# ntnu-arl/aerial_gym_simulator

Measured on AMD Instinct MI355X. Metric: env-steps/sec at N_envs=8192 per GPU (dynamics-only), higher is better.
Workload: dtype f32; 1 GPU; base_quadrotor position_setpoint_task, lee_position_control, empty_env, 1 sub-step/step (BASELINE configs[1]); num_envs_per_gpu=8192, num_envs_total=8192, rng=sync-free (device Philox4x32-10)

## Files before the change

aerial_gym_simulator_amd/csrc/agx_dynamics.hip:

```cpp
#include "agx_common.h"
#ifndef AGX_DYN_CONTRACT
#define AGX_DYN_CONTRACT 0
#endif
#ifndef AGX_DYN_WAVES
#define AGX_DYN_WAVES 3
#endif
#ifndef AGX_DYN_WAVES_LEAN_LAWS
#define AGX_DYN_WAVES_LEAN_LAWS 4
#endif
#ifndef AGX_DYN_WAVES_LOOP
#define AGX_DYN_WAVES_LOOP 2
#endif
#if AGX_DYN_CONTRACT
#pragma clang fp contract(fast)
#else
#pragma clang fp contract(off)
#endif
#include "agx_device_math.h"
#include "agx_nav_parts.h"
#include "agx_quad_math.h"
#include "agx_rng.h"
#include "agx_step_signal.h"

#include <chrono>
// ... 561 lines not shown
      }
      const bool any_dist = !body_wrench && (B.disturb != nullptr || B.disturb_prob > 0.0f);
      const bool split_root = !root_link && has_drag && any_dist;
      float dr[6] = {0.0f, 0.0f, 0.0f, 0.0f, 0.0f, 0.0f}, di[6] = {0.0f, 0.0f, 0.0f, 0.0f, 0.0f, 0.0f};
      if (has_drag) {
        float vbn = norm(d.vbody);
        dr[0] = (-P.lin_drag_linear[0] * d.vbody.x) + (-P.lin_drag_quadratic[0] * vbn * d.vbody.x);
        dr[1] = (-P.lin_drag_linear[1] * d.vbody.y) + (-P.lin_drag_quadratic[1] * vbn * d.vbody.y);
        dr[2] = (-P.lin_drag_linear[2] * d.vbody.z) + (-P.lin_drag_quadratic[2] * vbn * d.vbody.z);
        dr[3] = (-P.ang_drag_linear[0] * d.wbody.x) + (-P.ang_drag_quadratic[0] * fabsf(d.wbody.x) * d.wbody.x);
        dr[4] = (-P.ang_drag_linear[1] * d.wbody.y) + (-P.ang_drag_quadratic[1] * fabsf(d.wbody.y) * d.wbody.y);
        dr[5] = (-P.ang_drag_linear[2] * d.wbody.z) + (-P.ang_drag_quadratic[2] * fabsf(d.wbody.z) * d.wbody.z);
      }
      if (B.disturb) {
        const float *dd = B.disturb + (size_t)(sub_base + sub) * 7 * n + i;
        float occ = dd[0];
#pragma unroll
        for (int c = 0; c < 6; ++c) {
          float lo = -B.disturb_max[c], hi = B.disturb_max[c];
          di[c] = ((hi - lo) * dd[(size_t)(1 + c) * n] + lo) * occ;
        }
      } else if (B.disturb_prob > 0.0f) {
        float ud[7];
        rng_fill<7>(B.rng_seed, B.env_index_base + i, agx::step_index(B), RNG_DISTURB + sub_base + sub, ud);
        float occ = ud[0] < B.disturb_prob ? 1.0f : 0.0f;
#pragma unroll
        for (int c = 0; c < 6; ++c) {
          float lo = -B.disturb_max[c], hi = B.disturb_max[c];
          di[c] = ((hi - lo) * ud[1 + c] + lo) * occ;
        }
      }
      if (!body_wrench && (has_drag || any_dist)) {
#pragma unroll
        for (int c = 0; c < 6; ++c) bw[c] = split_root ? bw[c] + (dr[c] + di[c]) : (bw[c] + dr[c]) + di[c];
      }
      if (B.body_force && sub == k - 1) {
        AGX_AT(B.body_force, 0) = bw[0]; AGX_AT(B.body_force, 1) = bw[1]; AGX_AT(B.body_force, 2) = bw[2];
      }
      integrate(P, s, V3{bw[0], bw[1], bw[2]}, V3{bw[3], bw[4], bw[5]});
      if (B.boxes) {
        traj[(sub * 3 + 0) * bd + tid] = s.p.x;
        traj[(sub * 3 + 1) * bd + tid] = s.p.y;
        traj[(sub * 3 + 2) * bd + tid] = s.p.z;
        if (sub == 0) { tlo = s.p; thi = s.p; }
        tlo = V3{fminf(tlo.x, s.p.x), fminf(tlo.y, s.p.y), fminf(tlo.z, s.p.z)};
        thi = V3{fmaxf(thi.x, s.p.x), fmaxf(thi.y, s.p.y), fmaxf(thi.z, s.p.z)};
      }
    }
    bool crashed = crashed_in != 0;
    if (B.boxes && k > 0) crashed = collide_trajectory(B.boxes, B.num_boxes, n, i, traj, k, bd, tid, tlo, thi, P.collision_radius) || crashed;
    store_state(B.state, n, i, s);
    if (k > 0) {
      if (lean) store_body_velocities(B.derived, n, i, d);
      else store_derived(B.derived, n, i, d);
#pragma unroll
      for (int j = 0; j < M; ++j) AGX_AT(B.motor_thrust, j) = u[j];
      if (B.wrench_cmd) {
        AGX_AT(B.wrench_cmd, 0) = wc.f.x; AGX_AT(B.wrench_cmd, 1) = wc.f.y; AGX_AT(B.wrench_cmd, 2) = wc.f.z;
        AGX_AT(B.wrench_cmd, 3) = wc.t.x; AGX_AT(B.wrench_cmd, 4) = wc.t.y; AGX_AT(B.wrench_cmd, 5) = wc.t.z;
      }
    }
    float a_cur[AGX_MAX_ACTIONS], a_prev[AGX_MAX_ACTIONS];
#pragma unroll
    for (int c = 0; c < AGX_MAX_ACTIONS; ++c) {
      a_cur[c] = (k > 0 && !EXT) ? a_in[c] : a_old[c];
      a_prev[c] = (k >= 2 && !EXT) ? a_in[c] : ((k == 1 && !EXT) ? a_old[c] : a_prev_in[c]);
      if (c < A && k > 0 && !EXT && !lean) {
        AGX_AT(B.prev_actions, c) = a_prev[c];
        AGX_AT(B.actions, c) = a_cur[c];
      }
    }
    const int steps = steps_in + (more_launches ? 0 : 1);
    if (!more_launches) B.sim_steps[i] = steps;
    bool trunc = false;
    if (task_epilogue) {
      float rew;
      if (T.kind == AGX_TASK_POSITION) {
        rew = reward_position(s, d.qveh, d.wbody, tgt, crashed);
      } else {
        AGX_AT(T.prev_pos_err, 0) = ppe.x; AGX_AT(T.prev_pos_err, 1) = ppe.y; AGX_AT(T.prev_pos_err, 2) = ppe.z;
        V3 pe = quat_rotate_inverse(d.qveh, tgt - s.p);
        AGX_AT(T.pos_err, 0) = pe.x; AGX_AT(T.pos_err, 1) = pe.y; AGX_AT(T.pos_err, 2) = pe.z;
        rew = reward_navigation(T.rp, T.curriculum_progress, pe, ppe, a_cur[0], a_cur[2], a_cur[3], a_prev[0], a_prev[2],
                                a_prev[3], crashed);
      }
      T.reward[i] = rew;
      trunc = steps > T.episode_len;
      reset = (crashed && T.reset_on_collision) || trunc;
      B.reset_mask[i] = reset ? 1 : 0;
      if (T.successes) nav_bookkeeping_epilogue(T, i, true, tgt, s.p, crashed, trunc);
    }
    B.crashes[i] = crashed ? 1 : 0;
    if (!more_launches) B.truncations[i] = trunc ? 1 : 0;
  }
  if (T.kind != AGX_TASK_NONE && __ballot(reset) != 0ull && (tid & 63) == 0) atomicOr(B.reset_flag + B.flag_parity, 1);
  if (blockIdx.x == 0 && tid < 64) push_wait_finish(B, push_peek);
}

namespace q4 = quad;
AGX_DEV unsigned long long vote(bool p) { return __builtin_amdgcn_ballot_w64(p); }

struct QuadDerived {
  float euler, qveh, vveh, vbody, wbody;
};
AGX_DEV QuadDerived update_states_quad(float q, float v, float w, float extra, float &esn, float &ecs) {
  const int l = q4::lane_in_quad();
  QuadDerived d;
  const float e = q4::euler_xyz_0_2pi(q);
  d.euler = ssa(e);
  float sy, cy;
  const float half_yaw = (q4::bc<2>(e) * 1.0f) * 0.5f;
  sincos_bounded(l < 2 ? extra : half_yaw, sy, cy);
  esn = sy;
  ecs = cy;
  d.qveh = l == 2 ? sy : (l == 3 ? cy : 0.0f);
  d.vveh = q4::quat_rotate_inverse(d.qveh, v);
  d.vbody = q4::quat_rotate_inverse(q, v);
  d.wbody = q4::quat_rotate_inverse(q, w);
  return d;
}
AGX_DEV QuadDerived update_states_quad(float q, float v, float w) {
  float sn, cs;
  return update_states_quad(q, v, w, 0.0f, sn, cs);
}

template <int M>
struct QuadConsts {
  float grav, in0, in1, in2, ii0, ii1, ii2, pinv[M / 4][6], mapf[M], mapt[M], mass, dt;
};
template <int M>
AGX_DEV QuadConsts<M> load_quad_consts(const AgxRobotParams &P, const AgxRobotParams &S, int l, int l3) {
  QuadConsts<M> C;
  C.grav = P.gravity[l3];
  C.in0 = P.inertia[3 * l3 + 0]; C.in1 = P.inertia[3 * l3 + 1]; C.in2 = P.inertia[3 * l3 + 2];
  C.ii0 = P.inertia_inv[3 * l3 + 0]; C.ii1 = P.inertia_inv[3 * l3 + 1]; C.ii2 = P.inertia_inv[3 * l3 + 2];
#pragma unroll
  for (int h = 0; h < M / 4; ++h)
#pragma unroll
    for (int c = 0; c < 6; ++c) C.pinv[h][c] = P.alloc_pinv[6 * (l + 4 * h) + c];
  const float *wmap = S.root_link_mode != 0 ? P.alloc : P.wrench_map;
#pragma unroll
  for (int j = 0; j < M; ++j) {
    C.mapf[j] = wmap[M * l3 + j];
    C.mapt[j] = wmap[M * (3 + l3) + j];
  }
  C.mass = S.mass;
  C.dt = S.dt;
  return C;
}
template <int M>
AGX_DEV QuadConsts<M> load_quad_consts(const AgxRobotParams &P, int l, int l3) {
  return load_quad_consts<M>(P, P, l, l3);
}
AGX_DEV float quad_thrust_along_body_z(float q, float f, int l) {
  const float t1 = q * q4::bc<2>(q), t2 = q4::perm<1, 0, 2, 3>(q) * q4::bc<3>(q);
  const float c2a = 2.0f * (l == 1 ? t1 - t2 : t1 + t2);
  const float sqq = q * q;
  const float m22 = 1.0f - 2.0f * (q4::bc<0>(sqq) + q4::bc<1>(sqq));
  return q4::dot3(f, l == 2 ? m22 : c2a);
}
AGX_DEV float quad_desired_orientation_pos_vel_sc(float f, float sy, float cy, int l) {
  const float b3 = fdiv(f, q4::norm3(f));
  const float tmp = l == 0 ? cy : (l == 1 ? sy : 0.0f);
  const float cb = q4::cross3(b3, tmp);
  const float b2 = fdiv(cb, q4::norm3(cb));
  const float b1 = q4::cross3(b2, b3);
  return q4::rotmat_cols_to_quat(b1, b2, b3);
}
AGX_DEV float quad_desired_orientation_pos_vel(float f, float yaw, int l) {
  float sy, cy;
  sincos_bounded(yaw, sy, cy);
  return quad_desired_orientation_pos_vel_sc(f, sy, cy, l);
}
template <bool ZERO_RATE, int M>
AGX_DEV float quad_body_torque(const QuadConsts<M> &C, float q, float qd, float wb, float wsp, float kr, float kw, int l) {
  const float qe = q4::quat_mul(q4::conj(q), qd);
  const float pp = q4::rot1(qe) * q4::rot2(qe);
  const float pw = qe * q4::bc<3>(qe);
  const float mp = 2.0f * (pp + pw);
  const float mm = 2.0f * (pp - pw);
  const float rot_err = 0.5f * (l == 1 ? mm - mp : -(mp - mm));
  const float jw = (C.in0 * q4::bc<0>(wb) + C.in1 * q4::bc<1>(wb)) + C.in2 * q4::bc<2>(wb);
  const float ff = q4::cross3(wb, jw);
  const float we = ZERO_RATE ? wb : wb - q4::quat_rotate(qe, wsp);
  return ((-kr) * rot_err - kw * we) + ff;
}
template <int M>
AGX_DEV void quad_allocate(const AgxRobotParams &P, const QuadConsts<M> &C, float force, float torque, float (&u)[M / 4],
                           const float (&kT)[M / 4], const float (&tinc)[M / 4], const float (&tdec)[M / 4], float &fb, float &tb) {
  const float w0 = q4::bc<0>(force), w1 = q4::bc<1>(force), w2 = q4::bc<2>(force);
  const float w3 = q4::bc<0>(torque), w4 = q4::bc<1>(torque), w5 = q4::bc<2>(torque);
#pragma unroll
  for (int h = 0; h < M / 4; ++h) {
    float r = 0.0f;
    r += C.pinv[h][0] * w0;
    r += C.pinv[h][1] * w1;
    r += C.pinv[h][2] * w2;
    r += C.pinv[h][3] * w3;
    r += C.pinv[h][4] * w4;
    r += C.pinv[h][5] * w5;
    u[h] = motor_update(P, r, u[h], kT[h], tinc[h], tdec[h]);
  }
  fb = 0.0f;
  tb = 0.0f;
#pragma unroll
  for (int h = 0; h < M / 4; ++h) {
    const float u0 = q4::bc<0>(u[h]), u1 = q4::bc<1>(u[h]), u2 = q4::bc<2>(u[h]), u3 = q4::bc<3>(u[h]);
    fb += C.mapf[4 * h + 0] * u0; fb += C.mapf[4 * h + 1] * u1; fb += C.mapf[4 * h + 2] * u2; fb += C.mapf[4 * h + 3] * u3;
    tb += C.mapt[4 * h + 0] * u0; tb += C.mapt[4 * h + 1] * u1; tb += C.mapt[4 * h + 2] * u2; tb += C.mapt[4 * h + 3] * u3;
  }
}
template <int M>
AGX_DEV void quad_integrate(const AgxRobotParams &P, const QuadConsts<M> &C, float &p, float &q, float &v, float &w, float fb, float tb,
                            int l) {
  const float dt = C.dt;
  const float fw = q4::quat_rotate(q, fb);
  const float wbi = q4::quat_rotate_inverse(q, w);
  const float jwi = (C.in0 * q4::bc<0>(wbi) + C.in1 * q4::bc<1>(wbi)) + C.in2 * q4::bc<2>(wbi);
  const float rhs = tb - q4::cross3(wbi, jwi);
  const float dwb = (C.ii0 * q4::bc<0>(rhs) + C.ii1 * q4::bc<1>(rhs)) + C.ii2 * q4::bc<2>(rhs);
  const float wb_new = wbi + dt * dwb;
  float w_new = q4::quat_rotate(q, wb_new);
  float v_new = v + dt * fdiv(fw, C.mass);
  v_new = v_new + C.grav * dt;
  const float ml = fmaxf(1.0f - P.linear_damping * dt, 0.0f);
  const float ma = fmaxf(1.0f - P.angular_damping * dt, 0.0f);
  v_new = v_new * ml;
  w_new = w_new * ma;
  const float v2 = q4::dot3(v_new, v_new), w2 = q4::dot3(w_new, w_new);
  if (v2 > P.max_linear_velocity * P.max_linear_velocity) v_new = v_new * fdiv(P.max_linear_velocity, fsqrt(v2));
  if (w2 > P.max_angular_velocity * P.max_angular_velocity) w_new = w_new * fdiv(P.max_angular_velocity, fsqrt(w2));
  p = p + v_new * dt;
  const float wm2 = q4::dot3(w_new, w_new);
  if (wm2 != 0.0f) {
    const float wm = fsqrt(wm2);
    const float half = dt * wm * 0.5f;
    float sn, cs;
    sincos_bounded(half, sn, cs);
    const float sc = fdiv(sn, wm);
    const float x1 = w_new * sc;
    const float r3 = (x1 * q4::bc<3>(q) + q4::rot1(x1) * q4::rot2(q)) - q4::rot2(x1) * q4::rot1(q);
    const float xq = x1 * q;
    const float rw = (-q4::bc<0>(xq) - q4::bc<1>(xq)) - q4::bc<2>(xq);
    float rq = l == 3 ? rw : r3;
    rq += q * cs;
    const float nn = fsqrt(q4::dot4(rq, rq));
    q = fdiv(rq, nn);
  }
  v = v_new;
  w = w_new;
}

AGX_DEV float euler_rates_to_body_rates_quad(float euler, float rz) {
  const int l = q4::lane_in_quad();
  float sn, cs;
  sincos_bounded(euler, sn, cs);
  const float sr = q4::bc<0>(sn), cr = q4::bc<0>(cs), sp = q4::bc<1>(sn), cp = q4::bc<1>(cs);
  const float m0 = q4::by_lane(l, 1.0f, 0.0f, 0.0f);
  const float m1 = q4::by_lane(l, 0.0f, cr, -sr);
  const float m2 = q4::by_lane(l, -sp, sr * cp, cr * cp);
  return (m0 * 0.0f + m1 * 0.0f) + m2 * rz;
}
AGX_DEV float quat_from_euler_quad(float ang) {
  const int l = q4::lane_in_quad();
  float sn, cs;
  sincos_bounded(ang * 0.5f, sn, cs);
  const float sr = q4::bc<0>(sn), cr = q4::bc<0>(cs), sp = q4::bc<1>(sn), cp = q4::bc<1>(cs), sy = q4::bc<2>(sn), cy = q4::bc<2>(cs);
  const float a1 = l == 2 ? sy : cy, b1 = l == 0 ? sr : cr, c1 = l == 1 ? sp : cp;
  const float a2 = l == 2 ? cy : sy, b2 = l == 0 ? cr : sr, c2 = l == 1 ? cp : sp;
  const float t1 = a1 * b1 * c1, t2 = a2 * b2 * c2;
  return (l == 0 || l == 2) ? t1 - t2 : t1 + t2;
}

template <int CTRL, int M>
AGX_DEV void quad_controller(const AgxRobotParams &P, const QuadConsts<M> &C, float p, float q, float v, const QuadDerived &d, float a,
                             float a2, float kp, float kv, float kr, float kw, int l, float &force, float &torque) {
  const float yaw = q4::bc<2>(d.euler);
  float fz = 0.0f;
  if (CTRL == AGX_CTRL_FULLY_ACTUATED) {
    float nq = sqrtf(q4::dot4(a2, a2));
    nq = nq < 1e-9f ? 1e-9f : nq;
    const float qd = a2 / nq;
    const float acc = kp * (a - p) + kv * (0.0f - v);
    const float f = (acc - C.grav) * C.mass;
    force = q4::quat_rotate_inverse(q, f);
    torque = quad_body_torque<true>(C, q, qd, d.wbody, 0.0f, kr, kw, l);
    return;
  }
  if (CTRL == AGX_CTRL_POSITION || CTRL == AGX_CTRL_VELOCITY || CTRL == AGX_CTRL_VEL_STEERING) {
    float acc;
    if (CTRL == AGX_CTRL_POSITION) {
      acc = kp * (a - p) + kv * (0.0f - v);
    } else {
      const float sp_vel_w = q4::quat_rotate(d.qveh, a);
      acc = kp * (p - p) + kv * (sp_vel_w - v);
    }
    const float f = (acc - C.grav) * C.mass;
    fz = quad_thrust_along_body_z(q, f, l);
    const float qd = quad_desired_orientation_pos_vel(f, CTRL == AGX_CTRL_VELOCITY ? yaw : q4::bc<3>(a), l);
    if (CTRL == AGX_CTRL_POSITION) {
      torque = quad_body_torque<true>(C, q, qd, d.wbody, 0.0f, kr, kw, l);
    } else {
      float wsp = euler_rates_to_body_rates_quad(d.euler, CTRL == AGX_CTRL_VELOCITY ? q4::bc<3>(a) : 0.0f);
      if (l == 2) wsp = fminf(fmaxf(wsp, -P.max_yaw_rate), P.max_yaw_rate);
      torque = quad_body_torque<false>(C, q, qd, d.wbody, wsp, kr, kw, l);
    }
// ... 891 lines not shown
      if (l < 3) {
        AGX_QAT(B.derived, 0, ol) = d.euler;
        AGX_QAT(B.derived, 7, ol) = d.vveh;
        AGX_QAT(B.derived, 10, ol) = d.vbody;
        AGX_QAT(B.derived, 13, ol) = d.wbody;
      }
      AGX_QAT(B.derived, 3, ol) = d.qveh;
    }
    vbody = d.vbody;
    wbody = d.wbody;
  }
  if (valid) {
    float *o = obs + (size_t)i * 13;
    const float e = tgt - p;
    if (l < 3) { o[l] = e; o[7 + l] = vbody; o[10 + l] = wbody; }
    o[3 + l] = q;
    if (rows) {
      float *r = rows + (size_t)i * 16;
      if (B.push_world > 0) {
        const float e1 = q4::bc<1>(e), e2 = q4::bc<2>(e), q2 = q4::perm<0, 2, 2, 3>(q), q3 = q4::bc<3>(q);
        const float vb0 = q4::bc<0>(vbody), vb1 = q4::bc<1>(vbody), wb0 = q4::bc<0>(wbody), wb1 = q4::bc<1>(wbody), wb2 = q4::bc<2>(wbody);
        float t1 = 0.0f, t2 = 0.0f, t3 = 0.0f;
        if (l == 3) {
          t1 = tail_reward;
          t2 = tail_crashed ? 1.0f : 0.0f;
          t3 = tail_truncated ? 1.0f : 0.0f;
        }
        const float x0 = q4::by_lane(l, e, q, vb1, wb2);
        const float x1 = q4::by_lane(l, e1, q2, vbody, t1);
        const float x2 = q4::by_lane(l, e2, q3, wb0, t2);
        const float x3 = q4::by_lane(l, q, vb0, wb1, t3);
        row_store4_push(B, r + 4 * l, x0, x1, x2, x3);
      } else {
        if (l < 3) { row_store(B, r + l, e); row_store(B, r + 7 + l, vbody); row_store(B, r + 10 + l, wbody); }
        row_store(B, r + 3 + l, q);
        if (l == 0) {
          row_store(B, r + 13, tail_reward);
          row_store(B, r + 14, tail_crashed ? 1.0f : 0.0f);
          row_store(B, r + 15, tail_truncated ? 1.0f : 0.0f);
        }
      }
    }
  }
  step_rows_signal(B);
}
__global__ void __launch_bounds__(64, 1) k_reset_masked_quad_obs(AgxRobotParams P, AgxEnvBuffers B, int n, AgxResetArgs R,
                                                                 const float *__restrict__ target, float *__restrict__ obs) {
  reset_masked_quad_obs_body<false>(P, B, n, R, target, obs);
}
__global__ void __launch_bounds__(64, 1) k_reset_masked_quad_obs_host_draws(AgxRobotParams P, AgxEnvBuffers B, int n, AgxResetArgs R,
                                                                            const float *__restrict__ target,
                                                                            float *__restrict__ obs) {
  reset_masked_quad_obs_body<true>(P, B, n, R, target, obs);
}

#ifdef AGX_STEP_STAMPS
constexpr int kStampBlocks = 1024, kStampWords = 8;
__device__ unsigned long long g_step_stamps[kStampBlocks * 2 * kStampWords];
AGX_DEV void step_stamp(int k) {
  const unsigned long long t = k < 6 ? (unsigned long long)clock64() : (unsigned long long)wall_clock64();
  if ((threadIdx.x & 63u) == 0u && blockIdx.x < (unsigned)kStampBlocks)
    g_step_stamps[((size_t)blockIdx.x * 2 + (threadIdx.x >> 6)) * kStampWords + k] = t;
}
#define AGX_STAMP(k) step_stamp(k)
#define AGX_STAMP_ARRIVED(k) do { __builtin_amdgcn_s_waitcnt(0); step_stamp(k); } while (0)
#else
#define AGX_STAMP(k) do { } while (0)
#define AGX_STAMP_ARRIVED(k) do { } while (0)
#endif

AGX_DEV unsigned proof_key(float x) { return x >= 0.0f ? __float_as_uint(x) : 0x7FC00000u; }

__host__ __device__ inline unsigned proof_witness_bit(int episode_len, int reset_on_collision, int steps, float dist, float speed, float dt,
                                                      float vmax, float dv) {
  const int k = episode_len - steps + 1;
  if (k < 1 || k > AGX_PROOF_HORIZON || !(dist == dist) || !(speed == speed)) return 0u;
  bool w = k == 1 || !reset_on_collision;
  if (!w) {
    const float m = (float)(k - 1);
    const float travel = m * dt * fminf(vmax, speed + m * dv);
    w = dist + (travel * 1.01f + 1.0e-3f) < 8.0f;
  }
  return w ? (1u << k) : 0u;
}

template <bool MAX>
AGX_DEV unsigned wave_reduce_dpp(unsigned x) {
#define AGX_RED(ctrl)                                                                        \
  {                                                                                           \
    const unsigned y_ = (unsigned)__builtin_amdgcn_mov_dpp((int)x, (ctrl), 0xF, 0xF, true);   \
    x = MAX ? max(x, y_) : (x | y_);                                                          \
  }
  AGX_RED(0xB1)
  AGX_RED(0x4E)
  AGX_RED(0x124)
  AGX_RED(0x128)
#undef AGX_RED
  const unsigned r0 = (unsigned)__builtin_amdgcn_readlane((int)x, 0), r1 = (unsigned)__builtin_amdgcn_readlane((int)x, 16);
  const unsigned r2 = (unsigned)__builtin_amdgcn_readlane((int)x, 32), r3 = (unsigned)__builtin_amdgcn_readlane((int)x, 48);
  return MAX ? max(max(r0, r1), max(r2, r3)) : ((r0 | r1) | (r2 | r3));
}

AGX_DEV void proof_store_slot(const AgxTaskArgs &T, const AgxEnvBuffers &B, int wb, int nb, bool reset, unsigned horizon, int steps,
                              float dist, float speed) {
  const unsigned ar = wave_reduce_dpp<false>(reset ? 1u : 0u), hz = wave_reduce_dpp<false>(horizon);
  const unsigned ms = wave_reduce_dpp<true>((unsigned)max(steps, 0)), db = wave_reduce_dpp<true>(proof_key(dist));
  const unsigned vb = wave_reduce_dpp<true>(proof_key(speed));
  if ((threadIdx.x & 63u) == 0u) {
    uint4 *slot = reinterpret_cast<uint4 *>(T.proof_slots + ((size_t)(B.step_counter & 1) * nb + wb) * AGX_PROOF_SLOT_WORDS);
    slot[0] = make_uint4(((unsigned)B.step_counter + 1u) & 0x7FFFFFFFu, ar | (T.proof_mode == AGX_STEP_ANY ? 2u : 0u), hz, ms);
    slot[1] = make_uint4(db, vb, 0u, 0u);
  }
}

AGX_DEV void proof_fold_publish(const AgxTaskArgs &T, const AgxEnvBuffers &B, int nb) {
  const int lane = (int)(threadIdx.x & 63u);
  const uint32_t *bank = T.proof_slots + (size_t)((B.step_counter & 1) ^ 1) * nb * AGX_PROOF_SLOT_WORDS;
  unsigned t_and = 0x7FFFFFFFu, t_or = 0u, fl = 0u, hz = 0u, ms = 0u, db = 0u, vb = 0u;
  for (int b = lane; b < nb; b += 64) {
    const uint4 s0 = reinterpret_cast<const uint4 *>(bank + (size_t)b * AGX_PROOF_SLOT_WORDS)[0];
    const uint4 s1 = reinterpret_cast<const uint4 *>(bank + (size_t)b * AGX_PROOF_SLOT_WORDS)[1];
    t_and &= s0.x; t_or |= s0.x; fl |= s0.y; hz |= s0.z;
    ms = max(ms, s0.w); db = max(db, s1.x); vb = max(vb, s1.y);
  }
#pragma unroll
  for (int off = 32; off > 0; off >>= 1) {
    t_and &= (unsigned)__shfl_xor((int)t_and, off);
    t_or |= (unsigned)__shfl_xor((int)t_or, off);
    fl |= (unsigned)__shfl_xor((int)fl, off);
    hz |= (unsigned)__shfl_xor((int)hz, off);
    ms = max(ms, (unsigned)__shfl_xor((int)ms, off));
    db = max(db, (unsigned)__shfl_xor((int)db, off));
    vb = max(vb, (unsigned)__shfl_xor((int)vb, off));
  }
  if (lane != 0) return;
  const unsigned tag = t_and == t_or ? t_or : 0u;
  if (tag != 0u && (fl & 2u) && !(fl & 1u)) atomicAdd(T.proof_violation, 1u);
  uint32_t *h = T.proof_record;
  __hip_atomic_store(h + 7, tag, __ATOMIC_RELAXED, __HIP_MEMORY_SCOPE_SYSTEM);
  __builtin_amdgcn_fence(__ATOMIC_RELEASE, "wavefront");
  __builtin_amdgcn_s_waitcnt(0);
  __hip_atomic_store(h + 1, hz, __ATOMIC_RELAXED, __HIP_MEMORY_SCOPE_SYSTEM);
  __hip_atomic_store(h + 2, ms, __ATOMIC_RELAXED, __HIP_MEMORY_SCOPE_SYSTEM);
  __hip_atomic_store(h + 3, db, __ATOMIC_RELAXED, __HIP_MEMORY_SCOPE_SYSTEM);
  __hip_atomic_store(h + 4, vb, __ATOMIC_RELAXED, __HIP_MEMORY_SCOPE_SYSTEM);
  __hip_atomic_store(h + 5, fl, __ATOMIC_RELAXED, __HIP_MEMORY_SCOPE_SYSTEM);
  __builtin_amdgcn_fence(__ATOMIC_RELEASE, "wavefront");
  __builtin_amdgcn_s_waitcnt(0);
  __hip_atomic_store(h + 0, tag, __ATOMIC_RELAXED, __HIP_MEMORY_SCOPE_SYSTEM);
}

struct StepHandoff {
  float p[64], q[64], v[64], w[64];
  int reset[64];
};
template <int MODE>
AGX_DEV void position_step_quad(const AgxRobotParams &P0, const AgxEnvBuffers &B0, int n, const float *actions_in,
                                const AgxTaskArgs &T0, float *obs, StepHandoff *H) {
  constexpr bool FUSED = MODE != AGX_STEP_TWO;
  const int tid = threadIdx.x;
  AGX_STAMP(0); AGX_STAMP(6);
  AgxRobotParams P = P0;
  AgxEnvBuffers B = B0;
  AgxTaskArgs T = T0;
#define AGX_STEP_WAVE_ARGS(X)                                                                                                        \
  X(B, state) X(B, actions) X(B, prev_actions) X(B, motor_thrust) X(B, motor_kT) X(B, motor_tau_inc) X(B, motor_tau_dec)  \
  X(B, gains) X(B, wrench_cmd) X(B, crashes) X(B, truncations) X(B, sim_steps) X(B, reset_mask) X(B, reset_flag) X(B, flag_parity)    \
  X(B, step_counter) X(B, body_force)                                                                                                  \
  X(P, dt) X(P, dt_over_6) X(P, mass) X(P, min_thrust) X(P, max_thrust) X(P, max_rate) X(P, linear_damping) X(P, angular_damping)     \
  X(P, max_linear_velocity) X(P, max_angular_velocity) X(P, tau_inc_uniform) X(P, tau_dec_uniform)                                    \
  X(T, episode_len) X(T, target) X(T, reward) X(T, proof_slots) X(T, proof_violation) X(T, proof_dv)
  AGX_STEP_WAVE_ARGS(AGX_ARG_READ)
  AGX_ARG_READ(B, derived) AGX_ARG_READ(B, push_world)
  AGX_ARG_READ(P, root_link_mode) AGX_ARG_READ(P, use_rps) AGX_ARG_READ(P, use_discrete_approximation) AGX_ARG_READ(P, integration_rk4)
  AGX_ARG_READ(T, reset_on_collision) AGX_ARG_READ(T, kind) AGX_ARG_READ(T, proof_mode)
  const int grid_blocks = (int)gridDim.x;
  __builtin_amdgcn_sched_barrier(0);
  int env_blocks = grid_blocks - 1;
  int sw = (P_root_link_mode != 0 ? 1 : 0) | (P_use_rps != 0 ? 2 : 0) | (P_use_discrete_approximation != 0 ? 4 : 0) |
           (P_integration_rk4 != 0 ? 8 : 0) | (T_reset_on_collision != 0 ? 16 : 0) | ((T_kind & 0xFF) << 8) | ((T_proof_mode & 0xFF) << 16);
  arg_pin(n); arg_pin(actions_in);
  if (MODE == AGX_STEP_NONE) arg_pin(obs);
  AGX_STEP_WAVE_ARGS(AGX_ARG_PIN)
  if (MODE != AGX_STEP_ANY) { AGX_ARG_PIN(B, derived) }
  if (!FUSED) { AGX_ARG_PIN(B, push_world) }
  arg_pin(env_blocks);
#undef AGX_STEP_WAVE_ARGS
  arg_pin(sw);
  P.root_link_mode = sw & 1; P.use_rps = sw & 2; P.use_discrete_approximation = sw & 4; P.integration_rk4 = sw & 8;
  T.reset_on_collision = sw & 16; T.kind = (sw >> 8) & 0xFF; T.proof_mode = (sw >> 16) & 0xFF;
  const bool proof = T.proof_slots != nullptr;
  if (proof && blockIdx.x == 0) {
    proof_fold_publish(T0, B0, (int)gridDim.x - 1);
    AGX_STAMP(5); AGX_STAMP(7);
    return;
  }
  const int wb = (int)blockIdx.x - (proof ? 1 : 0);
  const int l = tid & 3, l3 = l < 3 ? l : 2;
  const int i = wb * 16 + (tid >> 2);
  const unsigned ol = ((unsigned)l * (unsigned)n + (unsigned)i) * 4u, ol3 = ((unsigned)l3 * (unsigned)n + (unsigned)i) * 4u;
  const bool valid = i < n;
  bool reset = false;
  if (FUSED && wb == 0 && tid == 0) B.reset_flag[B.flag_parity ^ 1] = 0;
  const bool push = !FUSED && wb == 0 && B.push_world > 0;
  uint32_t push_peek = 0u;
  if (__builtin_expect(push, false)) {
    push_publish_previous(B0);
    push_peek = push_wait_peek(B0);
  }
  float p = 0.0f, q = 0.0f, v = 0.0f, w = 0.0f, tgt = 0.0f, vbody = 0.0f, wbody = 0.0f;
  int steps = 0;
  float proof_dist = 0.0f, proof_speed = 0.0f;
  unsigned horizon = 0u;
  float u[1] = {0.0f}, a_in = 0.0f, a_old = 0.0f, fz = 0.0f, torque = 0.0f, dist = 0.0f;
  QuadDerived d{};
  bool crashed = false, trunc = false;
  AGX_STAMP(1);
  if (valid) {
    p = AGX_QAT(B.state, 0, ol3); q = AGX_QAT(B.state, 3, ol); v = AGX_QAT(B.state, 7, ol3); w = AGX_QAT(B.state, 10, ol3);
    u[0] = AGX_QAT(B.motor_thrust, 0, ol);
    float kT[1] = {1.0f}, tinc[1] = {P.tau_inc_uniform}, tdec[1] = {P.tau_dec_uniform};
    if (P.use_rps) kT[0] = AGX_QAT(B.motor_kT, 0, ol);
    if (B.motor_tau_inc) tinc[0] = AGX_QAT(B.motor_tau_inc, 0, ol);
    if (B.motor_tau_dec) tdec[0] = AGX_QAT(B.motor_tau_dec, 0, ol);
    a_in = actions_in[(size_t)i * 4 + l];
    a_old = AGX_QAT(B.actions, 0, ol);
    float kp = P0.gains_uniform[0 + l3], kv = P0.gains_uniform[3 + l3], kr = P0.gains_uniform[6 + l3], kw = P0.gains_uniform[9 + l3];
    if (B.gains) {
      kp = gain_load(&AGX_QAT(B.gains, 0, ol3)); kv = gain_load(&AGX_QAT(B.gains, 3, ol3));
      kr = gain_load(&AGX_QAT(B.gains, 6, ol3)); kw = gain_load(&AGX_QAT(B.gains, 9, ol3));
    }
    const int steps_in = B.sim_steps[i];
    tgt = T.kind == AGX_TASK_POSITION ? AGX_QAT(T.target, 0, ol3) : 0.0f;
    const QuadConsts<4> C = load_quad_consts<4>(P0, P, l, l3);
    AGX_STAMP_ARRIVED(2);

    const float a = clamp_minmax(a_in, -10.0f, 10.0f);
    float sy_sp, cy_sp;
    d = update_states_quad(q, v, w, q4::bc<3>(a), sy_sp, cy_sp);
    const float pe = a - p;
    const float ve = 0.0f - v;
    const float acc = kp * pe + kv * ve;
    const float f = (acc - C.grav) * C.mass;
    fz = quad_thrust_along_body_z(q, f, l);
    const float qd = quad_desired_orientation_pos_vel_sc(f, sy_sp, cy_sp, l);
    torque = quad_body_torque<true>(C, q, qd, d.wbody, 0.0f, kr, kw, l);

    float fb, tb;
    quad_allocate<4>(P, C, l == 2 ? fz : 0.0f, torque, u, kT, tinc, tdec, fb, tb);
    if (B.body_force && l < 3) AGX_QAT(B.body_force, 0, ol) = fb;
    quad_integrate(P, C, p, q, v, w, fb, tb, l);

    steps = steps_in + 1;
    if (T.kind == AGX_TASK_POSITION) {
      const float pe_t = q4::quat_apply(q4::conj(d.qveh), tgt - p);
      dist = q4::norm3(pe_t);
      if (dist > 8.0f) crashed = true;
      trunc = steps > T.episode_len;
      reset = (crashed && T.reset_on_collision) || trunc;
    }
  }
  AGX_STAMP(3);
  if (MODE == AGX_STEP_ANY) {
    H->p[tid] = p; H->q[tid] = q; H->v[tid] = v; H->w[tid] = w;
    H->reset[tid] = reset ? 1 : 0;
    __syncthreads();
  }
  AGX_STAMP(4);
  if (valid) {
    float rew = 0.0f;
    if (T.kind == AGX_TASK_POSITION) {
      const float ex = exp_cw((l == 0 ? -8.0f : -4.0f) * dist * dist);
      const float pos_reward = 3.0f * q4::bc<0>(ex) + 2.0f * q4::bc<1>(ex);
      const float dist_reward = (20.0f - dist) / 40.0f;
      const float axis_z = l == 2 ? 1.0f : 0.0f;
      const float up = q4::bc<2>(q4::quat_rotate(q, axis_z));
      const float tilt = fabsf(1.0f - up);
      const float spin = q4::norm3(d.wbody);
      const float quo = (1.0f / (l == 0 ? 0.1f + tilt * tilt : 1.0f + spin * spin)) * (l == 0 ? 0.2f : 3.0f);
      const float up_reward = q4::bc<0>(quo);
      const float ang_reward = q4::bc<1>(quo);
      float total = pos_reward + dist_reward + pos_reward * (up_reward + ang_reward);
      total = 1.0f * total;
      if (crashed) total = -20.0f;
      rew = total;
      proof_dist = dist;
    }
    if (proof) {
      proof_speed = q4::norm3(v);
      if (l == 0 && !reset && T.kind == AGX_TASK_POSITION) horizon = proof_witness_bit(T.episode_len, T.reset_on_collision, steps, proof_dist, proof_speed, P.dt, P.max_linear_velocity,
                                    T.proof_dv);
    }

    const bool own = MODE != AGX_STEP_ANY || !reset;
    if (own) {
      if (l < 3) AGX_QAT(B.state, 0, ol) = p;
      AGX_QAT(B.state, 3, ol) = q;
      if (l < 3) {
        AGX_QAT(B.state, 7, ol) = v;
        AGX_QAT(B.state, 10, ol) = w;
      }
      AGX_QAT(B.motor_thrust, 0, ol) = u[0];
    }
    if (MODE != AGX_STEP_ANY) {
      if (l < 3) {
        AGX_QAT(B.derived, 0, ol) = d.euler;
        AGX_QAT(B.derived, 7, ol) = d.vveh;
        AGX_QAT(B.derived, 10, ol) = d.vbody;
        AGX_QAT(B.derived, 13, ol) = d.wbody;
      }
      AGX_QAT(B.derived, 3, ol) = d.qveh;
    }
    vbody = d.vbody;
    wbody = d.wbody;
    if (B.wrench_cmd) {
      if (l < 3) {
        AGX_QAT(B.wrench_cmd, 0, ol) = l == 2 ? fz : 0.0f;
        AGX_QAT(B.wrench_cmd, 3, ol) = torque;
      }
    }
    AGX_QAT(B.prev_actions, 0, ol) = a_old;
    AGX_QAT(B.actions, 0, ol) = a_in;
    if (l == 0) {
      if (own) B.sim_steps[i] = steps;
      if (T.kind == AGX_TASK_POSITION) {
        T.reward[i] = rew;
        B.reset_mask[i] = reset ? 1 : 0;
      }
      B.crashes[i] = crashed ? 1 : 0;
      B.truncations[i] = trunc ? 1 : 0;
    }
  }
  const bool some = __ballot(reset) != 0ull;
  if (T.kind != AGX_TASK_NONE && some && (tid & 63) == 0) {
    atomicOr(B.reset_flag + B.flag_parity, 1);
    if (MODE == AGX_STEP_NONE) atomicAdd(T.proof_violation, 1u);
  }
  if (proof) proof_store_slot(T, B, wb, env_blocks, reset, horizon, steps, proof_dist, proof_speed);
  if (!FUSED) {
    if (__builtin_expect(push, false)) push_wait_finish(B0, push_peek);
    AGX_STAMP(5); AGX_STAMP(7);
    return;
  }
  if (MODE == AGX_STEP_ANY) {
    AGX_STAMP(5); AGX_STAMP(7);
    return;
  }
  if (valid) {
    float *o = obs + (size_t)i * 13;
    const float e = tgt - p;
    if (l < 3) { o[l] = e; o[7 + l] = vbody; o[10 + l] = wbody; }
    o[3 + l] = q;
  }
  AGX_STAMP(5); AGX_STAMP(7);
}

AGX_DEV void position_step_helper(const AgxRobotParams &P0, const AgxEnvBuffers &B0, int n, const AgxTaskArgs &T0, const AgxResetArgs &R0,
                                  float *obs, const StepHandoff *H) {
  AGX_STAMP(0); AGX_STAMP(6);
  AgxRobotParams P = P0;
  AgxEnvBuffers B = B0;
  AgxTaskArgs T = T0;
  AgxResetArgs R = R0;
#define AGX_HELPER_WAVE_ARGS(X, XN)                                                                                                  \
  X(B, sim_steps) X(B, episode_count) X(B, env_index_base) X(B, bounds_min) X(B, bounds_max) X(B, state) X(B, derived) X(B, gains)    \
  X(B, motor_tau_inc) X(B, motor_tau_dec) X(B, motor_thrust) X(B, motor_kT)                                                           \
  X(P, use_rps) X(P, min_thrust) X(P, max_thrust) X(T, kind) X(T, episode_len) X(T, target) X(T, proof_slots)                         \
  XN(R, lower_bound_min, 3) XN(R, lower_bound_max, 3) XN(R, upper_bound_min, 3) XN(R, upper_bound_max, 3) XN(R, min_state, 13)        \
  XN(R, max_state, 13) XN(R, gains_min, 12) XN(R, gains_max, 12) X(R, tau_inc_min) X(R, tau_inc_max) X(R, tau_dec_min)                \
  X(R, tau_dec_max) X(R, kT_min) X(R, kT_max) X(R, randomize_gains) X(R, seed)
  AGX_HELPER_WAVE_ARGS(AGX_ARG_READ, AGX_ARG_READ_N)
  arg_pin(n); arg_pin(obs);
  AGX_HELPER_WAVE_ARGS(AGX_ARG_PIN, AGX_ARG_PIN_N)
#undef AGX_HELPER_WAVE_ARGS
  const bool proof = T.proof_slots != nullptr;
  if (proof && blockIdx.x == 0) return;
  const int lane = (int)(threadIdx.x & 63u);
  const int wb = (int)blockIdx.x - (proof ? 1 : 0);
  const int l = lane & 3, l3 = l < 3 ? l : 2;
  const int i = wb * 16 + (lane >> 2);
  const unsigned ol = ((unsigned)l * (unsigned)n + (unsigned)i) * 4u, ol3 = ((unsigned)l3 * (unsigned)n + (unsigned)i) * 4u;
  const bool valid = i < n;
  int steps_in = 0, ep = 0;
  float tgt = 0.0f;
  AGX_STAMP(1);
  if (valid) {
    steps_in = B.sim_steps[i];
    if (B.episode_count) ep = B.episode_count[i];
    tgt = T.kind == AGX_TASK_POSITION ? AGX_QAT(T.target, 0, ol3) : 0.0f;
  }
  AGX_STAMP_ARRIVED(2);
  const bool early = valid && T.kind == AGX_TASK_POSITION && steps_in + 1 > T.episode_len;
  ResetValues<4> V{};
  if (vote(early) != 0ull) {
    ResetDraws<4> D{};
    wave_reset_draws<4>(R, B.env_index_base + i, ep, early && l == 0, D);
    V = reset_env_values<4>(P, R, D);
  }
  AGX_STAMP(3);
  __syncthreads();
  AGX_STAMP(4);
  float p = H->p[lane], q = H->q[lane], v = H->v[lane], w = H->w[lane];
  const bool mine = H->reset[lane] != 0;
  const bool late = mine && !early;
  if (vote(late) != 0ull) {
    ResetDraws<4> D{};
    wave_reset_draws<4>(R, B.env_index_base + i, ep, late && l == 0, D);
    const ResetValues<4> V2 = reset_env_values<4>(P, R, D);
    if (late) V = V2;
  }
  if (vote(mine) != 0ull) {
    if (mine && l == 0) reset_env_store<4>(P, B, n, R, i, ep, V);
    const EnvState &s = V.s;
    const float npv = q4::by_lane(l3, q4::bc<0>(s.p.x), q4::bc<0>(s.p.y), q4::bc<0>(s.p.z));
    const float nq = q4::by_lane(l, q4::bc<0>(s.q.x), q4::bc<0>(s.q.y), q4::bc<0>(s.q.z), q4::bc<0>(s.q.w));
    const float nv = q4::by_lane(l3, q4::bc<0>(s.v.x), q4::bc<0>(s.v.y), q4::bc<0>(s.v.z));
    const float nw = q4::by_lane(l3, q4::bc<0>(s.w.x), q4::bc<0>(s.w.y), q4::bc<0>(s.w.z));
    p = mine ? npv : p; q = mine ? nq : q; v = mine ? nv : v; w = mine ? nw : w;
  }
  const QuadDerived d2 = update_states_quad(q, v, w);
  if (valid) {
    if (l < 3) {
      AGX_QAT(B.derived, 0, ol) = d2.euler;
      AGX_QAT(B.derived, 7, ol) = d2.vveh;
      AGX_QAT(B.derived, 10, ol) = d2.vbody;
      AGX_QAT(B.derived, 13, ol) = d2.wbody;
    }
    AGX_QAT(B.derived, 3, ol) = d2.qveh;
    float *o = obs + (size_t)i * 13;
    const float e = tgt - p;
    if (l < 3) { o[l] = e; o[7 + l] = d2.vbody; o[10 + l] = d2.wbody; }
    o[3 + l] = q;
  }
  AGX_STAMP(5); AGX_STAMP(7);
}

__global__ void __launch_bounds__(64, 1)
    k_env_step_quad_position(AgxRobotParams P, AgxEnvBuffers B, int n, const float *__restrict__ actions_in, AgxTaskArgs T) {
  position_step_quad<AGX_STEP_TWO>(P, B, n, actions_in, T, nullptr, nullptr);
}

template <int MODE>
__global__ void __launch_bounds__(MODE == AGX_STEP_ANY ? 128 : 64, 1)
    k_position_step_fused(AgxRobotParams P, AgxEnvBuffers B, int n, const float *__restrict__ actions_in, AgxTaskArgs T, AgxResetArgs R,
                          float *__restrict__ obs) {
  if constexpr (MODE == AGX_STEP_ANY) {
    __shared__ StepHandoff H;
    if (__builtin_amdgcn_readfirstlane((int)(threadIdx.x >> 6)) == 0) position_step_quad<MODE>(P, B, n, actions_in, T, obs, &H);
    else position_step_helper(P, B, n, T, R, obs, &H);
  } else {
    position_step_quad<MODE>(P, B, n, actions_in, T, obs, nullptr);
  }
}

#ifdef AGX_STEP_STAMPS
}
extern "C" int agx_debug_step_stamps(unsigned long long *out, int blocks) {
  if (blocks < 0 || blocks > agx::kStampBlocks) return -1;
  return (int)hipMemcpyFromSymbol(out, HIP_SYMBOL(agx::g_step_stamps), sizeof(unsigned long long) * 2 * agx::kStampWords * (size_t)blocks);
}
namespace agx {
#endif

__global__ void __launch_bounds__(256) k_reset_assets(AgxEnvBuffers B, int n, int K, AgxResetArgs R, const float *__restrict__ u1,
                                                       const float *__restrict__ u2, const float *__restrict__ u_sel,
                                                       const float *__restrict__ min_ratio, const float *__restrict__ max_ratio,
                                                       int num_obstacles, int nk, float *__restrict__ asset_state) {
  const int env = blockIdx.x;
  const int a = blockIdx.y * blockDim.x + threadIdx.x;
  if (a >= K) return;
  if (B.reset_flag[B.flag_parity] == 0 || B.reset_mask[env] == 0) return;
  reset_asset_one(B, R, env, a, K, u1, u2, u_sel, min_ratio, max_ratio, num_obstacles, nk, asset_state);
}

}

using namespace agx;

#define AGX_DISPATCH_M(M_, ...)                                       \
  switch (M_) {                                                       \
    case 4: { constexpr int kM = 4; __VA_ARGS__; } break;             \
    case 6: { constexpr int kM = 6; __VA_ARGS__; } break;             \
    case 8: { constexpr int kM = 8; __VA_ARGS__; } break;             \
    default: return fail(AGX_E_UNSUPPORTED, "num_motors %d: kernels are built for 4, 6 and 8 motors", M_); \
  }
#define AGX_DISPATCH_CTRL(C_, ...)                                                         \
  switch (C_) {                                                                            \
    case AGX_CTRL_NONE: { constexpr int kC = AGX_CTRL_NONE; __VA_ARGS__; } break;          \
    case AGX_CTRL_POSITION: { constexpr int kC = AGX_CTRL_POSITION; __VA_ARGS__; } break;  \
    case AGX_CTRL_VELOCITY: { constexpr int kC = AGX_CTRL_VELOCITY; __VA_ARGS__; } break;  \
    case AGX_CTRL_ATTITUDE: { constexpr int kC = AGX_CTRL_ATTITUDE; __VA_ARGS__; } break;  \
    case AGX_CTRL_RATES: { constexpr int kC = AGX_CTRL_RATES; __VA_ARGS__; } break;        \
    case AGX_CTRL_ACCELERATION: { constexpr int kC = AGX_CTRL_ACCELERATION; __VA_ARGS__; } break; \
    case AGX_CTRL_VEL_STEERING: { constexpr int kC = AGX_CTRL_VEL_STEERING; __VA_ARGS__; } break; \
    case AGX_CTRL_FULLY_ACTUATED: { constexpr int kC = AGX_CTRL_FULLY_ACTUATED; __VA_ARGS__; } break; \
    case AGX_CTRL_WRENCH: { constexpr int kC = AGX_CTRL_WRENCH; __VA_ARGS__; } break;      \
    default: return fail(AGX_E_ARG, "unknown controller id %d", C_);                       \
  }

static int check_common(const AgxRobotParams *P, const AgxEnvBuffers *B, int n) {
  AGX_REQUIRE(B != nullptr, "null buffers");
  AGX_REQUIRE(n > 0, "num_envs must be > 0 (got %d)", n);
  AGX_REQUIRE(n <= (1 << 26), "num_envs %d above 2^26 = 67 108 864 per GPU: shard the job (the SoA accesses use 32-bit byte offsets)", n);
  AGX_REQUIRE(B->flag_parity == 0 || B->flag_parity == 1, "flag_parity must be 0 or 1");
  AGX_REQUIRE((!B->step_rows[0] && !B->step_rows[1]) ||
                  (B->step_rows[0] && B->step_rows[1] && B->step_reward && B->crashes && B->truncations),
              "step_rows needs both parity buffers, step_reward, crashes and truncations");
  if (P) {
    AGX_REQUIRE(P->num_motors >= 1 && P->num_motors <= AGX_MAX_MOTORS, "num_motors out of range");
    AGX_REQUIRE(P->num_actions >= 1 && P->num_actions <= AGX_MAX_ACTIONS, "num_actions out of range");
    AGX_REQUIRE(P->controller >= 0 && P->controller <= AGX_CTRL_WRENCH, "unknown controller id %d", P->controller);
    AGX_REQUIRE(P->controller != AGX_CTRL_FULLY_ACTUATED || P->num_actions == 7, "fully actuated controller needs 7 actions");
    AGX_REQUIRE(P->controller != AGX_CTRL_NONE || P->num_actions == P->num_motors, "no_control needs num_actions == num_motors");
    AGX_REQUIRE(P->controller == AGX_CTRL_NONE || P->controller == AGX_CTRL_FULLY_ACTUATED || P->controller == AGX_CTRL_WRENCH ||
                    P->num_actions == 4,
                "Lee controllers take 4 actions");
  }
  return AGX_OK;
}

static bool quad_kernel_usable(const AgxRobotParams *P, const AgxEnvBuffers *B, const AgxTaskArgs *T) {
  if (!option_env_step_quad() || B->boxes || B->launch_flags != 0 || B->disturb || B->disturb_prob > 0.0f || P->num_actions != 4) return false;
  if (T->kind != AGX_TASK_NONE && T->kind != AGX_TASK_POSITION) return false;
  for (int c = 0; c < 3; ++c)
    if (P->lin_drag_linear[c] != 0.0f || P->lin_drag_quadratic[c] != 0.0f || P->ang_drag_linear[c] != 0.0f ||
        P->ang_drag_quadratic[c] != 0.0f)
      return false;
  return true;
}

static bool quad_loop_kernel_usable(const AgxRobotParams *P, const AgxEnvBuffers *B, int n, int k) {
  if (!option_env_step_quad() || pick_block(n) != 64 || k < 1 || B->launch_flags != 0) return false;
  const bool lee_quad = P->num_motors == 4 && P->num_actions == 4 && P->controller >= AGX_CTRL_POSITION &&
                        P->controller <= AGX_CTRL_VEL_STEERING;
  const bool fa_octa = P->num_motors == 8 && P->num_actions == 7 && P->controller == AGX_CTRL_FULLY_ACTUATED;
  const bool lee_octa = P->num_motors == 8 && P->num_actions == 4 && (P->controller == AGX_CTRL_POSITION || P->controller == AGX_CTRL_VELOCITY);
  if (!lee_quad && !fa_octa && !lee_octa) return false;
  for (int c = 0; c < 3; ++c)
    if (P->lin_drag_linear[c] != 0.0f || P->lin_drag_quadratic[c] != 0.0f || P->ang_drag_linear[c] != 0.0f ||
        P->ang_drag_quadratic[c] != 0.0f)
      return false;
  return true;
}

template <int M, int CTRL, bool WIDE>
static void launch_env_step(int k, int n, int block, size_t lds, hipStream_t stream, const AgxRobotParams &P, const AgxEnvBuffers &B,
                            const float *actions_in, const AgxTaskArgs &T) {
  if (k == 1)
    hipLaunchKernelGGL((k_env_step<M, CTRL, true, WIDE>), dim3(blocks_for(n, block)), dim3(block), lds, stream, P, B, n, actions_in, k, T);
  else
    hipLaunchKernelGGL((k_env_step<M, CTRL, false, WIDE>), dim3(blocks_for(n, block)), dim3(block), lds, stream, P, B, n, actions_in, k, T);
}

extern "C" int agx_env_step(const AgxRobotParams *P, const AgxEnvBuffers *B, int n, const float *actions_in, int k,
                            const AgxTaskArgs *task, void *stream) {
  if (int e = check_common(P, B, n)) return e;
  AGX_REQUIRE(P != nullptr, "null params");
  AGX_REQUIRE(actions_in != nullptr, "null actions");
  AGX_REQUIRE(k >= 0 && k <= AGX_MAX_SUBSTEPS, "k_substeps out of range: %d", k);
  AGX_REQUIRE(P->controller != AGX_CTRL_WRENCH || k <= 1,
              "external controller (AGX_CTRL_WRENCH): one launch per physics sub-step, the host re-evaluates the controller in between");
  AGX_REQUIRE((B->launch_flags & ~0xFF0F) == 0, "launch_flags: bits 0-3 and the sub-step index in bits 8-15");
  AGX_REQUIRE((B->launch_flags & AGX_LAUNCH_BODY_WRENCH) == 0 || P->controller == AGX_CTRL_WRENCH,
              "AGX_LAUNCH_BODY_WRENCH (external robot) goes with AGX_CTRL_WRENCH: actions_in is a wrench [N][6]");
  AGX_REQUIRE((B->launch_flags & 4) == 0 || ((B->launch_flags & 3) == 0 && P->controller != AGX_CTRL_WRENCH &&
                                             (!task || task->kind != AGX_TASK_NAVIGATION)),
              "AGX_LAUNCH_LEAN needs the fused step of a built-in controller without the navigation reward (it reads the action history)");
  AGX_REQUIRE(B->state && B->derived && B->actions && B->prev_actions && B->motor_thrust && B->crashes && B->truncations &&
                  B->sim_steps,
              "null env buffer");
  AGX_REQUIRE(!P->use_rps || B->motor_kT, "null motor_kT with use_rps");
  AgxTaskArgs T{};
  if (task) T = *task;
  AGX_REQUIRE(T.kind >= AGX_TASK_NONE && T.kind <= AGX_TASK_NAVIGATION, "bad task kind %d", T.kind);
  if (T.kind != AGX_TASK_NONE) {
    AGX_REQUIRE(T.target && T.reward && B->reset_mask && B->reset_flag, "null task buffer");
    AGX_REQUIRE(T.kind != AGX_TASK_NAVIGATION || (T.pos_err && T.prev_pos_err && P->num_actions >= 4), "null navigation buffer");
    AGX_REQUIRE((!T.successes && !T.timeouts && !T.counters) || (T.successes && T.timeouts && T.counters && T.kind == AGX_TASK_NAVIGATION),
                "navigation bookkeeping in the epilogue needs successes, timeouts and counters, and the navigation task kind");
  }
  const int block = pick_block(n);
  const size_t lds = B->boxes ? (size_t)k * 3 * block * sizeof(float) : 0;
  if (k == 1 && block == 64 && P->num_motors == 4 && P->controller == AGX_CTRL_POSITION && quad_kernel_usable(P, B, &T)) {
    hipLaunchKernelGGL(k_env_step_quad_position, dim3(blocks_for(n, 16) + (T.proof_slots ? 1 : 0)), dim3(64), 0, (hipStream_t)stream, *P,
                       *B, n, actions_in, T);
    return check_launch("agx_env_step");
  }
  AGX_REQUIRE(!T.proof_slots && T.proof_mode == AGX_STEP_TWO, "AgxTaskArgs.proof_*: the four-lanes-per-env position kernel only");
  if (quad_loop_kernel_usable(P, B, n, k)) {
    const size_t lds4 = B->boxes ? (size_t)k * 3 * 16 * sizeof(float) : 0;
    if (P->num_motors == 8 && P->controller == AGX_CTRL_POSITION) {
      hipLaunchKernelGGL((k_env_step_quad_loop<8, AGX_CTRL_POSITION>), dim3(blocks_for(n, 16)), dim3(64), lds4, (hipStream_t)stream, *P, *B, n,
                         actions_in, k, T);
      return check_launch("agx_env_step");
    }
    if (P->num_motors == 8 && P->controller == AGX_CTRL_VELOCITY) {
      hipLaunchKernelGGL((k_env_step_quad_loop<8, AGX_CTRL_VELOCITY>), dim3(blocks_for(n, 16)), dim3(64), lds4, (hipStream_t)stream, *P, *B, n,
                         actions_in, k, T);
      return check_launch("agx_env_step");
    }
    switch (P->controller) {
#define AGX_QUAD_LOOP(C_)                                                                                                        \
// ... 430 lines not shown
```

Measured before the change: 1.010 billion env-steps/s.

## Move vehicle-frame yaw quaternion and reset decision into helper wave in fused step

In the two-wave fused position step, the helper wave now computes the yaw-only vehicle quaternion from the pre-step orientation and passes it through shared memory. It also recomputes the reset/crash decision itself instead of reading a reset flag from the main wave. The main wave skips the full update_states_quad, computing only the yaw sincos and body angular rate, and defers its distance/crash check until after the barrier. The helper also reads kernel arguments straight from the kernarg segment, hardcodes proof mode to true, and pins the constants with inline asm and a sched barrier. The aim is to shorten the critical path of the main dynamics wave by shifting work onto the otherwise idle helper wave. The costs are a second crash computation, tighter coupling through the kernarg struct layout, and a proof flag that is now always on.

```diff
diff --git a/aerial_gym_simulator_amd/csrc/agx_dynamics.hip b/aerial_gym_simulator_amd/csrc/agx_dynamics.hip
--- a/aerial_gym_simulator_amd/csrc/agx_dynamics.hip
+++ b/aerial_gym_simulator_amd/csrc/agx_dynamics.hip
@@ -737,6 +737,11 @@
 AGX_DEV QuadConsts<M> load_quad_consts(const AgxRobotParams &P, int l, int l3) {
   return load_quad_consts<M>(P, P, l, l3);
 }
+AGX_DEV void quad_consts_keep(const QuadConsts<4> &C) {
+  asm volatile("" ::"v"(C.grav), "v"(C.in0), "v"(C.in1), "v"(C.in2), "v"(C.ii0), "v"(C.ii1), "v"(C.ii2), "v"(C.pinv[0][0]),
+               "v"(C.pinv[0][1]), "v"(C.pinv[0][2]), "v"(C.pinv[0][3]), "v"(C.pinv[0][4]), "v"(C.pinv[0][5]), "v"(C.mapf[0]),
+               "v"(C.mapf[1]), "v"(C.mapf[2]), "v"(C.mapf[3]), "v"(C.mapt[0]), "v"(C.mapt[1]), "v"(C.mapt[2]), "v"(C.mapt[3]));
+}
 AGX_DEV float quad_thrust_along_body_z(float q, float f, int l) {
   const float t1 = q * q4::bc<2>(q), t2 = q4::perm<1, 0, 2, 3>(q) * q4::bc<3>(q);
   const float c2a = 2.0f * (l == 1 ? t1 - t2 : t1 + t2);
@@ -1934,7 +1939,7 @@
 
 struct StepHandoff {
   float p[64], q[64], v[64], w[64];
-  int reset[64];
+  float qveh[64];
 };
 template <int MODE>
 AGX_DEV void position_step_quad(const AgxRobotParams &P0, const AgxEnvBuffers &B0, int n, const float *actions_in,
@@ -2015,11 +2020,20 @@
     const int steps_in = B.sim_steps[i];
     tgt = T.kind == AGX_TASK_POSITION ? AGX_QAT(T.target, 0, ol3) : 0.0f;
     const QuadConsts<4> C = load_quad_consts<4>(P0, P, l, l3);
+    if (MODE == AGX_STEP_ANY) {
+      __builtin_amdgcn_sched_barrier(0);
+      quad_consts_keep(C);
+    }
     AGX_STAMP_ARRIVED(2);
 
     const float a = clamp_minmax(a_in, -10.0f, 10.0f);
     float sy_sp, cy_sp;
-    d = update_states_quad(q, v, w, q4::bc<3>(a), sy_sp, cy_sp);
+    if (MODE == AGX_STEP_ANY) {
+      sincos_bounded(q4::bc<3>(a), sy_sp, cy_sp);
+      d.wbody = q4::quat_rotate_inverse(q, w);
+    } else {
+      d = update_states_quad(q, v, w, q4::bc<3>(a), sy_sp, cy_sp);
+    }
     const float pe = a - p;
     const float ve = 0.0f - v;
     const float acc = kp * pe + kv * ve;
@@ -2034,7 +2048,7 @@
     quad_integrate(P, C, p, q, v, w, fb, tb, l);
 
     steps = steps_in + 1;
-    if (T.kind == AGX_TASK_POSITION) {
+    if (MODE != AGX_STEP_ANY && T.kind == AGX_TASK_POSITION) {
       const float pe_t = q4::quat_apply(q4::conj(d.qveh), tgt - p);
       dist = q4::norm3(pe_t);
       if (dist > 8.0f) crashed = true;
@@ -2045,10 +2059,17 @@
   AGX_STAMP(3);
   if (MODE == AGX_STEP_ANY) {
     H->p[tid] = p; H->q[tid] = q; H->v[tid] = v; H->w[tid] = w;
-    H->reset[tid] = reset ? 1 : 0;
     __syncthreads();
+    d.qveh = H->qveh[tid];
   }
   AGX_STAMP(4);
+  if (MODE == AGX_STEP_ANY && valid && T.kind == AGX_TASK_POSITION) {
+    const float pe_t = q4::quat_apply(q4::conj(d.qveh), tgt - p);
+    dist = q4::norm3(pe_t);
+    if (dist > 8.0f) crashed = true;
+    trunc = steps > T.episode_len;
+    reset = (crashed && T.reset_on_collision) || trunc;
+  }
   if (valid) {
     float rew = 0.0f;
     if (T.kind == AGX_TASK_POSITION) {
@@ -2138,7 +2159,7 @@
 }
 
 AGX_DEV void position_step_helper(const AgxRobotParams &P0, const AgxEnvBuffers &B0, int n, const AgxTaskArgs &T0, const AgxResetArgs &R0,
-                                  float *obs, const StepHandoff *H) {
+                                  float *obs, StepHandoff *H) {
   AGX_STAMP(0); AGX_STAMP(6);
   AgxRobotParams P = P0;
   AgxEnvBuffers B = B0;
@@ -2147,15 +2168,19 @@
 #define AGX_HELPER_WAVE_ARGS(X, XN)                                                                                                  \
   X(B, sim_steps) X(B, episode_count) X(B, env_index_base) X(B, bounds_min) X(B, bounds_max) X(B, state) X(B, derived) X(B, gains)    \
   X(B, motor_tau_inc) X(B, motor_tau_dec) X(B, motor_thrust) X(B, motor_kT)                                                           \
-  X(P, use_rps) X(P, min_thrust) X(P, max_thrust) X(T, kind) X(T, episode_len) X(T, target) X(T, proof_slots)                         \
+  X(P, use_rps) X(P, min_thrust) X(P, max_thrust) X(T, episode_len) X(T, target)                                                      \
   XN(R, lower_bound_min, 3) XN(R, lower_bound_max, 3) XN(R, upper_bound_min, 3) XN(R, upper_bound_max, 3) XN(R, min_state, 13)        \
   XN(R, max_state, 13) XN(R, gains_min, 12) XN(R, gains_max, 12) X(R, tau_inc_min) X(R, tau_inc_max) X(R, tau_dec_min)                \
   X(R, tau_dec_max) X(R, kT_min) X(R, kT_max) X(R, randomize_gains) X(R, seed)
   AGX_HELPER_WAVE_ARGS(AGX_ARG_READ, AGX_ARG_READ_N)
+  AGX_ARG_READ(T, kind) AGX_ARG_READ(T, reset_on_collision)
+  int sw = (T_kind & 0xFF) | (T_reset_on_collision != 0 ? 0x100 : 0);
   arg_pin(n); arg_pin(obs);
   AGX_HELPER_WAVE_ARGS(AGX_ARG_PIN, AGX_ARG_PIN_N)
 #undef AGX_HELPER_WAVE_ARGS
-  const bool proof = T.proof_slots != nullptr;
+  arg_pin(sw);
+  T.kind = sw & 0xFF; T.reset_on_collision = sw & 0x100;
+  constexpr bool proof = true;
   if (proof && blockIdx.x == 0) return;
   const int lane = (int)(threadIdx.x & 63u);
   const int wb = (int)blockIdx.x - (proof ? 1 : 0);
@@ -2164,9 +2189,10 @@
   const unsigned ol = ((unsigned)l * (unsigned)n + (unsigned)i) * 4u, ol3 = ((unsigned)l3 * (unsigned)n + (unsigned)i) * 4u;
   const bool valid = i < n;
   int steps_in = 0, ep = 0;
-  float tgt = 0.0f;
+  float tgt = 0.0f, q0 = 0.0f;
   AGX_STAMP(1);
   if (valid) {
+    q0 = AGX_QAT(B.state, 3, ol);
     steps_in = B.sim_steps[i];
     if (B.episode_count) ep = B.episode_count[i];
     tgt = T.kind == AGX_TASK_POSITION ? AGX_QAT(T.target, 0, ol3) : 0.0f;
@@ -2179,11 +2205,21 @@
     wave_reset_draws<4>(R, B.env_index_base + i, ep, early && l == 0, D);
     V = reset_env_values<4>(P, R, D);
   }
+  float qveh;
+  {
+    const float e = q4::euler_xyz_0_2pi(q0);
+    float sy, cy;
+    const float half_yaw = (q4::bc<2>(e) * 1.0f) * 0.5f;
+    sincos_bounded(half_yaw, sy, cy);
+    qveh = l == 2 ? sy : (l == 3 ? cy : 0.0f);
+  }
+  H->qveh[lane] = qveh;
   AGX_STAMP(3);
   __syncthreads();
   AGX_STAMP(4);
   float p = H->p[lane], q = H->q[lane], v = H->v[lane], w = H->w[lane];
-  const bool mine = H->reset[lane] != 0;
+  const float dist = q4::norm3(q4::quat_apply(q4::conj(qveh), tgt - p));
+  const bool mine = early || (valid && T.kind == AGX_TASK_POSITION && dist > 8.0f && T.reset_on_collision);
   const bool late = mine && !early;
   if (vote(late) != 0ull) {
     ResetDraws<4> D{};
@@ -2222,6 +2258,15 @@
   position_step_quad<AGX_STEP_TWO>(P, B, n, actions_in, T, nullptr, nullptr);
 }
 
+struct PositionStepKernargs {
+  AgxRobotParams P;
+  AgxEnvBuffers B;
+  int n;
+  const float *actions_in;
+  AgxTaskArgs T;
+  AgxResetArgs R;
+  float *obs;
+};
 template <int MODE>
 __global__ void __launch_bounds__(MODE == AGX_STEP_ANY ? 128 : 64, 1)
     k_position_step_fused(AgxRobotParams P, AgxEnvBuffers B, int n, const float *__restrict__ actions_in, AgxTaskArgs T, AgxResetArgs R,
@@ -2229,7 +2274,13 @@
   if constexpr (MODE == AGX_STEP_ANY) {
     __shared__ StepHandoff H;
     if (__builtin_amdgcn_readfirstlane((int)(threadIdx.x >> 6)) == 0) position_step_quad<MODE>(P, B, n, actions_in, T, obs, &H);
-    else position_step_helper(P, B, n, T, R, obs, &H);
+    else {
+      typedef const PositionStepKernargs __attribute__((address_space(4))) *kernarg_ptr;
+      kernarg_ptr A = (kernarg_ptr)__builtin_amdgcn_kernarg_segment_ptr();
+      asm volatile("" : "+s"(A));
+      const PositionStepKernargs *G = (const PositionStepKernargs *)A;
+      position_step_helper(G->P, G->B, G->n, G->T, G->R, G->obs, &H);
+    }
   } else {
     position_step_quad<MODE>(P, B, n, actions_in, T, obs, nullptr);
   }
```

Result: slower. 967.4 million env-steps/s (-4.2%).
